# GoogleCloudPlatform/plspm-python

Measured on AMD Instinct MI355X. Metric: bootstrap replicates/sec (6-LV satisfaction model, N=10k), higher is better.
Workload: dtype f64

## Files before the change

plspm-python_amd/csrc/solver_wave16.h:

```cpp
#pragma once
#include "solver_wave.h"

namespace plspm {

template <int LMAX> struct W16 { static constexpr int VP = LMAX + 1; static constexpr bool TCOPY = LMAX <= 8; };

template <int LMAX>
struct Wave16Ws {
    double* stage;
    double* V;
    double* w;
    double* mu;
    double *Qm, *Gm, *Em;
    double* a;
    double* sink;
    double* scr;
    double* inv;
};
template <int LMAX> PLSPM_HD constexpr long wave16_v_doubles() {
    return (W16<LMAX>::TCOPY ? 2 : 1) * 64 * W16<LMAX>::VP > 16 * 66 ? (W16<LMAX>::TCOPY ? 2 : 1) * 64 * W16<LMAX>::VP : 16 * 66;
}
template <int LMAX> PLSPM_HD constexpr long wave16_ws_doubles(int L, int kmax, int n_chol = 0) { return wave16_v_doubles<LMAX>() + 64 + 64 + 3 * LMAX * LMAX + 2 * LMAX + (long)L * regression_scratch_doubles(kmax) + n_chol / 2; }
template <int LMAX> PLSPM_HD void wave16_carve(Wave16Ws<LMAX>& ws, double* base, int L, int kmax) {
    static_assert(LMAX == 32 || LMAX == 16 || LMAX == 8, "pair lane: column t mod LMAX, rows t / LMAX + (64 / LMAX) u");
    double* p = base;
    ws.stage = p; ws.V = p; p += wave16_v_doubles<LMAX>();
    ws.w = p; p += 64; ws.mu = p; p += 64;
    ws.Qm = p; p += LMAX * LMAX; ws.Gm = p; p += LMAX * LMAX; ws.Em = p; p += LMAX * LMAX;
    ws.a = p; p += LMAX; ws.sink = p; p += LMAX;
    ws.scr = p; p += (long)L * regression_scratch_doubles(kmax);
    ws.inv = p;
}
template <int LMAX> PLSPM_HD bool wave16_solver_covers(int P, int L, int n_chol, int kmax) {
    return P >= 1 && P <= 64 && L > LMAX / 2 && L <= LMAX && n_chol / 2 <= 16 * 66 && wave16_ws_doubles<LMAX>(L, kmax, n_chol) * (long)sizeof(double) <= (LMAX > 16 ? 53 : 40) * 1024;
}

struct NmWaveIo {
    double* maps;
    int force_T;
    int* steps;
    double bound_scale = 1.0;
};

template <int LMAX, bool MODEB = false, bool NM = false, class Ex>
PLSPM_HD void solve_problem_wave16(Ex& ex, const ModelDesc& md, const Wave16Ws<LMAX>& ws, const double* Md, const FitOutputs& out, const NmWaveIo* io = nullptr, double* nmk = nullptr) {
    constexpr int PMAX = 64, NE = LMAX * LMAX / 64;
    const int P = md.P, L = md.L, PS = cov_ld(P), t = ex.tid, p = t;
    const bool valid = p < P;
    const int pc = valid ? p : P - 1;
    const int lp = md.lvof[pc];
    const int em = t % LMAX, er0 = t / LMAX;
    const bool lvlane = t < L;
    unsigned dsc[NE];
#pragma unroll
    for (int u = 0; u < NE; ++u) {
        const int el = er0 + (64 / LMAX) * u;
        const bool pr = el < L && em < L;
        const int elc = pr ? el : 0, emc = pr ? em : 0;
        const int b0 = md.boff[elc];
        dsc[u] = (unsigned)b0 | (unsigned)(pr ? md.boff[elc + 1] - b0 : 0) << 8 | (unsigned)(pr ? (int)md.C[elc * L + emc] + 2 * (int)md.C[emc * L + elc] : 0) << 16 |
                 (pr ? 1u : 0u) << 24;
    }
    unsigned dl[NE];
#pragma unroll
    for (int u = 0; u < NE; ++u) dl[u] = dsc[u];
    auto pb0 = [&](int u) { return (int)(dl[u] & 255u); };
    auto pk = [&](int u) { return (int)((dl[u] >> 8) & 255u); };
    auto dlm = [&](int u) { return (int)((dl[u] >> 16) & 3u); };
    auto pairu = [&](int u) { return (dl[u] >> 24) != 0u; };
    int nk = 0;
    unsigned fpack = 0u;
    if (lvlane) {
        const int o = md.pred_off[t];
        nk = md.pred_off[t + 1] - o;
        for (int r = 0; r < 4; ++r) if (r < nk) fpack |= (unsigned)md.pred_idx[o + r] << (8 * r);
    }
    const int ne = md.n_eff;
    const double shp = md.scaled ? md.shift[pc] : 0.0;
    int kbmax = 0, kbB = 0;
    unsigned long long ends = 0ull;
    for (int l = 0; l < L; ++l) {
        const int k = md.boff[l + 1] - md.boff[l];
        kbmax = k > kbmax ? k : kbmax;
        if (MODEB && md.mode[l] == MODE_B) kbB = k > kbB ? k : kbB;
        ends |= 1ull << (md.boff[l + 1] - 1);
    }
    ends = ex.uniform(ends);
    bool singular = false;

    ex.mark(0);
    double s[PMAX];
    double dpp = 0.0, mup = 0.0;
    const double n = ex.uniform_d(Md[(long)P * PS + P]);
    ex.template load_cov<PMAX>(Md, PS, P, s, ws.stage, mup, dpp);
    if (!valid) { mup = 0.0; dpp = 0.0; }
    ex.mark(1);
    const double inv_n = ex.uniform_d(1.0 / n);
    const double sdraw = NM ? nm_column_sd(dpp * inv_n, mup * inv_n) : 1.0;
    ws.mu[p] = mup;
    ws.w[p] = NM ? (valid ? sdraw : 1.0) : 1.0;
    ex.sync();
    double fac = inv_n;
    if (!NM && md.scaled) {
        const double tot = ex.allsum(valid ? mup + n * shp : 0.0);
        const double np_ = n * (double)P, grand = tot / np_;
        const double d = shp - grand;
        const double ss = ex.allsum(valid ? dpp + 2.0 * d * mup + n * d * d : 0.0);
        const double g2 = ss / (np_ - 1.0) * ((n - 1.0) / n);
        fac = ex.uniform_d(1.0 / (n * g2));
    }
    ex.fence();
#pragma unroll
    for (int qb = 0; qb < PMAX; qb += 8) {
#pragma unroll
        for (int q = qb; q < qb + 8; ++q) {
            double v;
            if constexpr (NM) v = ((s[q] - (mup * ex.bcast(mup, (q < P) ? q : P - 1, ws.mu)) * inv_n) * inv_n) / (sdraw * ex.bcast(sdraw, (q < P) ? q : P - 1, ws.w));
            else v = (s[q] - (mup * ex.bcast(mup, (q < P) ? q : P - 1, ws.mu)) * inv_n) * fac;
            s[q] = (q < P) ? v : 0.0;
        }
        ex.pin8(s[qb], s[qb + 1], s[qb + 2], s[qb + 3], s[qb + 4], s[qb + 5], s[qb + 6], s[qb + 7]);
    }
    if (!valid) {
#pragma unroll
        for (int q = 0; q < PMAX; ++q) s[q] = 0.0;
    }
    const double sdp = NM ? sqrt(((dpp - (mup * mup) * inv_n) * inv_n) / (sdraw * sdraw)) : treated_sd(dpp, mup, inv_n, fac);
    if constexpr (!NM) {
        if (ex.vote_any(valid && sdp == 0.0)) {
            const double keep = (sdp == 0.0) ? 0.0 : 1.0;
#pragma unroll
            for (int q = 0; q < PMAX; ++q) s[q] *= keep;
        }
    }
    const double corr2 = ex.uniform_d(n / (n - 1.0));
    ex.mark(2);

    const bool modeb = MODEB && valid && md.mode[lp] == MODE_B;
    const int bb0 = md.boff[lp], bk = md.boff[lp + 1] - bb0, bi = p - bb0;
    const long boffB = modeb ? md.chol_off[lp] / 2 : 0;
    if constexpr (MODEB) {
        ex.sync();
        ws.mu[p] = (sdp > 0.0) ? sdp * sdp : 1e300;
        double* A = (kbB & 1) ? ws.stage : ws.inv;
        double* An = (kbB & 1) ? ws.inv : ws.stage;
        auto fill_block = [&](double* dst) {
#pragma unroll
            for (int q = 0; q < PMAX; ++q)
                if (modeb && q >= bb0 && q < bb0 + bk) dst[boffB + bi * bk + (q - bb0)] = s[q];
        };
        auto fill_block_all = [&](double* dst) {
            double* mine_row = dst + boffB + bi * bk - bb0;
            double* junk = ws.stage + 2 * LMAX * 16 + p;
            const unsigned bkm = modeb ? (unsigned)bk : 0u;
#pragma unroll
            for (int q = 0; q < PMAX; ++q) {
                double* d = ((unsigned)(q - bb0) < bkm) ? mine_row + q : junk;
                *d = s[q];
            }
        };
        bool okrow = true;
        ex.mark(20);
        auto sweep_rows = [&](auto krc) {
            constexpr int KR = decltype(krc)::value;
            fill_block_all(ws.inv);
            ex.sync();
            ex.mark(21);
            double row[KR];
            {
                const double* Ib0 = ws.inv + boffB + bi * bk;
#pragma unroll
                for (int c = 0; c < KR; ++c) row[c] = (modeb && c < bk) ? Ib0[c] : 0.0;
            }
            ex.mark(22);
            for (int j = 0; j < kbB; ++j) {
                double* Pj = ws.stage + ((j & 1) * LMAX + lp) * 16;
                if (modeb && bi == j) {
#pragma unroll
                    for (int c = 0; c < KR; ++c) Pj[c] = row[c];
                }
                ex.sync();
                if (modeb && j < bk) {
                    double f = 0.0;
#pragma unroll
                    for (int c = 0; c < KR; ++c) f = (c == j) ? row[c] : f;
                    const double piv = Pj[j];
                    okrow = okrow && (piv > PLSPM_PIVOT_RTOL * ws.mu[bb0 + j]);
                    const double ip = wave_rcp(piv);
                    const bool pivlane = bi == j;
                    const double fip = f * ip;
#pragma unroll
                    for (int c = 0; c < KR; ++c) {
                        const double rjc = Pj[c] * ip;
                        const double off = pivlane ? rjc : row[c] - f * rjc;
                        const double dia = pivlane ? ip : -fip;
                        row[c] = (c == j) ? dia : off;
                    }
                }
            }
            ex.mark(23);
#pragma unroll
            for (int c = 0; c < KR; ++c) if (modeb && c < bk) ws.inv[boffB + bi * bk + c] = row[c];
            ex.sync();
            ex.mark(24);
        };
        if (kbB <= 8) sweep_rows(std::integral_constant<int, 8>{});
        else if (kbB <= 12) sweep_rows(std::integral_constant<int, 12>{});
        else if (kbB <= 16) sweep_rows(std::integral_constant<int, 16>{});
        else {
        fill_block(A);
        ex.sync();
        for (int j = 0; j < kbB; ++j) {
            if (modeb) {
                const double* Ab = A + boffB;
                double* Ob = An + boffB;
                if (j < bk) {
                    const double piv = Ab[j * bk + j];
                    okrow = okrow && (piv > PLSPM_PIVOT_RTOL * ws.mu[bb0 + j]);
                    const double ip = 1.0 / piv;
                    const double f = Ab[bi * bk + j];
                    for (int c = 0; c < bk; ++c) {
                        const double rjc = Ab[j * bk + c] * ip;
                        double v;
                        if (bi == j) v = (c == j) ? ip : rjc;
                        else v = (c == j) ? -f * ip : Ab[bi * bk + c] - f * rjc;
                        Ob[bi * bk + c] = v;
                    }
                } else {
                    for (int c = 0; c < bk; ++c) Ob[bi * bk + c] = Ab[bi * bk + c];
                }
            }
            ex.sync();
            double* t = A; A = An; An = t;
        }
        }
        const bool any_bad = ex.vote_any(modeb && !okrow);
        for (int l = 0; any_bad && l < L; ++l) {
            if (md.mode[l] != MODE_B) continue;
            const int k = md.boff[l + 1] - md.boff[l];
            const bool bad_here = ex.vote_any(modeb && lp == l && !okrow);
            if (!bad_here) continue;
            if (lp == l) fill_block(ws.inv);
            ex.sync();
            if (p == l) {
                double* F = ws.inv + md.chol_off[l] / 2;
                bool ok = k > 1 && jacobi_pinv(F, k, ws.stage);
                if (!ok) singular = true;
                for (int r = 0; r < k; ++r) for (int c = 0; c < r; ++c) F[r * k + c] = F[c * k + r];
            }
            ex.sync();
        }
        ex.mark(25);
    }


    const int* fglob = md.pred_idx + (lvlane ? md.pred_off[t] : 0);
    const long rscr = regression_scratch_doubles(md.kmax);
    const int km = md.kmax;
    auto pred = [&](int r) { return r < 4 ? (int)((fpack >> (8 * r)) & 255u) : fglob[r]; };
    auto regress = [&](const double* M) {
        double* scratch = ws.scr + t * rscr;
        double* x = scratch + 2 * km * km;
        bool ok;
        if (nk <= 4) {
            unsigned fp = fpack;
            ex.opaque(fp);
            ok = wave_ldl4(M, LMAX, fp, nk, t, x);
        } else {
            for (int r = 0; r < nk; ++r) {
                for (int c = 0; c < nk; ++c) scratch[r * nk + c] = M[fglob[r] * LMAX + fglob[c]];
                x[r] = M[fglob[r] * LMAX + t];
            }
            ok = chol_factor(scratch, nk);
            if (ok) chol_solve(scratch, nk, x);
        }
        if (!ok && !(nk > 1 && pinv_solve(M, LMAX, fglob, nk, t, x, scratch))) singular = true;
        return x;
    };

    const double icorr2 = ex.uniform_d((n - 1.0) / n);
    double Qe[NE], wp = valid ? 1.0 : 0.0;
#pragma unroll
    for (int u = 0; u < NE; ++u) Qe[u] = 0.0;
    int iteration = 0, phase = 0;
    double a_prev = 0.0, Ra_prev = 0.0;
    if constexpr (NM) {
        ex.sync();
        wp = valid ? 1.0 / sqrt((double)(md.boff[lp + 1] - md.boff[lp])) : 0.0;
        ws.w[p] = valid ? wp : 1.0;
        ex.sync();
        phase = 1;
    }
    while (true) {
        int pl = p, lpl = lp;
        ex.opaque(pl); ex.opaque(lpl);
#pragma unroll
        for (int u = 0; u < NE; ++u) { dl[u] = dsc[u]; ex.opaque(dl[u]); }
        const int eml = pl % LMAX, er0l = pl / LMAX;
        ex.mark(16);
        if constexpr (W16<LMAX>::TCOPY) ex.template seg_products2<PMAX, 64 * W16<LMAX>::VP * 8>(s, ws.w, P, ends, ws.V + pl * W16<LMAX>::VP, wp);
        else ex.template seg_products<PMAX>(s, ws.w, P, ends, valid ? ws.V + pl * W16<LMAX>::VP : ex.sink(ws.sink));
        ex.mark(17);
        ex.sync();
        ex.mark(18);
        if constexpr (NE == 1) {
            double s0 = 0.0, s1 = 0.0;
            int pb = pb0(0);
            ex.opaque(pb);
            const double* vv = ws.V + pb * W16<LMAX>::VP + eml;
            const double* ww = ws.w + pb;
            for (int i0 = 0; i0 < kbmax; i0 += 8) {
                double v[8];
#pragma unroll
                for (int j = 0; j < 8; ++j) {
                    if constexpr (W16<LMAX>::TCOPY) v[j] = (i0 + j < pk(0)) ? vv[(64 + i0 + j) * W16<LMAX>::VP] : 0.0;
                    else v[j] = (i0 + j < pk(0)) ? ww[i0 + j] * vv[(i0 + j) * W16<LMAX>::VP] : 0.0;
                }
                s0 += v[0]; s1 += v[1]; s0 += v[2]; s1 += v[3]; s0 += v[4]; s1 += v[5]; s0 += v[6]; s1 += v[7];
            }
            Qe[0] = s0 + s1;
            ws.Qm[pl] = pairu(0) ? Qe[0] : 1.0;
        } else {
            double s0[NE], s1[NE];
#pragma unroll
            for (int u = 0; u < NE; ++u) { s0[u] = 0.0; s1[u] = 0.0; }
            auto terms = [&](auto ttc) {
                constexpr int TT = decltype(ttc)::value;
                for (int i0 = 0; i0 < kbmax; i0 += TT) {
#pragma unroll
                    for (int u = 0; u < NE; ++u) {
                        if ((64 / LMAX) * u < L) {
                            const int pb = pb0(u), pkk = pk(u);
                            const double* vv = ws.V + pb * W16<LMAX>::VP + eml;
                            const double* ww = ws.w + pb;
                            double v[TT];
#pragma unroll
                            for (int j = 0; j < TT; ++j) v[j] = (i0 + j < pkk) ? ww[i0 + j] * vv[(i0 + j) * W16<LMAX>::VP] : 0.0;
#pragma unroll
                            for (int j = 0; j < TT; j += 2) { s0[u] += v[j]; s1[u] += v[j + 1]; }
                        }
                    }
                }
            };
            if (kbmax <= (NE <= 4 ? 4 : 2)) terms(std::integral_constant<int, (NE <= 4 ? 4 : 2)>{});
            else if (NE > 4) terms(std::integral_constant<int, 4>{});
            else {
#pragma unroll
                for (int u = 0; u < NE; ++u) {
                    if ((64 / LMAX) * u < L) {
                        int pb = pb0(u);
                        ex.opaque(pb);
                        const int pkk = pk(u);
                        const double* vv = ws.V + pb * W16<LMAX>::VP + eml;
                        const double* ww = ws.w + pb;
                        for (int i0 = 0; i0 < kbmax; i0 += 8) {
                            double v[8];
#pragma unroll
                            for (int j = 0; j < 8; ++j) v[j] = (i0 + j < pkk) ? ww[i0 + j] * vv[(i0 + j) * W16<LMAX>::VP] : 0.0;
                            s0[u] += v[0]; s1[u] += v[1]; s0[u] += v[2]; s1[u] += v[3]; s0[u] += v[4]; s1[u] += v[5]; s0[u] += v[6]; s1[u] += v[7];
                        }
                    }
                }
            }
#pragma unroll
            for (int u = 0; u < NE; ++u) {
                if ((64 / LMAX) * u < L) {
                    Qe[u] = s0[u] + s1[u];
                    ws.Qm[pl + 64 * u] = pairu(u) ? Qe[u] : 1.0;
                }
            }
        }
        ex.sync();
        ex.mark(19);
        bool nm_first = false;
        if constexpr (NM) {
            nm_first = iteration == 0;
            const double wfl = nm_first ? 1.0 : wave_rsqrt(ws.Qm[lpl * LMAX + lpl]);
            const double a_cur = valid ? wp * wfl : 0.0, Ra_cur = valid ? ws.V[pl * W16<LMAX>::VP + lpl] * wfl : 0.0;
            bool stop = false;
            double ub = 0.0;
            if (!nm_first) {
                const double d = a_cur - a_prev, Rd = Ra_cur - Ra_prev;
                ub = n * ex.allsum(d * Rd);
                stop = (io && io->force_T > 0) ? (iteration >= io->force_T) : (ub * (io ? io->bound_scale : 1.0) < md.tol * (1.0 - 1e-9));
                if (iteration > md.max_iter) stop = true;
            }
            if (stop) break;
            a_prev = a_cur; Ra_prev = Ra_cur;
            const double cmap = a_cur / sdraw;
            if (io && io->maps && valid) io->maps[(long)iteration * (P + L + 1) + pl] = cmap;
            if (io && io->maps && pl == 0) io->maps[(long)iteration * (P + L + 1) + P + L] = ub;
            nmk[pl] = valid ? (mup * inv_n) * cmap : 0.0;
        }
        if (!NM && phase == 2) break;
        if (phase == 0) {
            wp = valid ? wave_rsqrt(ws.Qm[lpl * LMAX + lpl]) : 0.0;
            ws.w[pl] = valid ? wp : 1.0;
            ex.sync();
            ex.mark(3);
            phase = 1;
            continue;
        }
        ++iteration;
        ex.mark(9);
        const double rm = wave_rsqrt(ws.Qm[eml * LMAX + eml]), am = NM ? (nm_first ? 1.0 : rm) : rm * icorr2;
#pragma unroll
        for (int u = 0; u < NE; ++u) {
            if ((64 / LMAX) * u < L) {
                const int ell = er0l + (64 / LMAX) * u;
                const double rl = wave_rsqrt(ws.Qm[ell * LMAX + ell]), al = NM ? (nm_first ? 1.0 : rl) : rl * icorr2;
                const double Ge = al * am * Qe[u];
                double Ee = 0.0;
                if (pairu(u)) {
                    if (md.scheme == SCHEME_PATH) {
                        if (dlm(u) & 1) Ee = Qe[u] * rl * rm;
                    } else if (dlm(u)) {
                        const int d = (dlm(u) & 1) + (dlm(u) >> 1);
                        Ee = (md.scheme == SCHEME_CENTROID) ? ((Ge > 0.0) ? 1.0 : ((Ge < 0.0) ? -1.0 : 0.0)) : Ge * corr2 * (double)d;
                    }
                    ws.Gm[pl + 64 * u] = Ge; ws.Em[pl + 64 * u] = al * Ee;
                    if (ell == eml) ws.a[ell] = al;
                }
            }
        }
        ex.sync();
        ex.mark(10);
        if constexpr (NM) {
            if (io && io->maps && lvlane) {
                double k0 = 0.0;
                for (int q = md.boff[pl]; q < md.boff[pl + 1]; ++q) k0 += nmk[q];
                io->maps[(long)(iteration - 1) * (P + L + 1) + P + pl] = -k0;
            }
        }
        if (md.scheme == SCHEME_PATH) {
            if (lvlane && nk > 0) {
                const double* x = regress(ws.Gm);
#pragma unroll
                for (int r = 0; r < 4; ++r) if (r < nk) ws.Em[pred(r) * LMAX + pl] = ws.a[pred(r)] * x[r];
                for (int r = 4; r < nk; ++r) ws.Em[pred(r) * LMAX + pl] = ws.a[pred(r)] * x[r];
            }
            ex.sync();
        }
        ex.mark(11);
        double c0 = 0.0, c1 = 0.0;
#pragma unroll
        for (int m = 0; m + 1 < LMAX; m += 2) {
            if (m < L) c0 += ws.V[pl * W16<LMAX>::VP + m] * ws.Em[m * LMAX + lpl];
            if (m + 1 < L) c1 += ws.V[pl * W16<LMAX>::VP + m + 1] * ws.Em[(m + 1) * LMAX + lpl];
        }
        double wn = valid ? c0 + c1 : 0.0;
        if constexpr (MODEB) {
            ws.mu[pl] = wn;
            ex.sync();
            if (modeb) {
                const double* Ib = ws.inv + boffB + bi * bk;
                const double* cb = ws.mu + bb0;
                double a0 = 0.0, a1 = 0.0;
                int q = 0;
                for (; q + 1 < bk; q += 2) { a0 += Ib[q] * cb[q]; a1 += Ib[q + 1] * cb[q + 1]; }
                if (q < bk) a0 += Ib[q] * cb[q];
                wn = a0 + a1;
            }
        }
        if constexpr (NM) {
            wp = wn;
            ws.w[pl] = valid ? wp : 1.0;
            ex.sync();
            ex.mark(12);
        } else {
        const double dd = fabs(wp) - fabs(wn);
        const double conv = ex.allsum(dd * dd);
        wp = wn;
        ws.w[pl] = valid ? wp : 1.0;
        ex.sync();
        ex.mark(12);
        if (conv < md.tol || iteration > md.max_iter) phase = 2;
        }
    }
    const bool not_converged = iteration > md.max_iter;
    ex.mark(4);

    const double wfp = wave_rsqrt(ws.Qm[lp * LMAX + lp]);
    wp *= wfp;
    unsigned negmask = 0u;
    {
        double vr[LMAX];
#pragma unroll
        for (int l = 0; l < LMAX; ++l) vr[l] = ws.V[p * W16<LMAX>::VP + (l < L ? l : 0)];
#pragma unroll
        for (int l = 0; l < LMAX; ++l)
            if (!NM && l < L) { const int neg = ex.vote_count(valid && vr[l] < 0.0 && sdp != 0.0); if (P - 2 * neg < 0) negmask |= 1u << l; }
    }
    const double sgl = ((negmask >> lp) & 1u) ? -1.0 : 1.0;
    const double vlp = ws.V[p * W16<LMAX>::VP + lp];
    double* const Cs = ws.Gm;
    double* const Bm = ws.Em;
    double* const Ind = ws.Qm;
    {
        const double wfm = wave_rsqrt(ws.Qm[em * LMAX + em]), sm = ((negmask >> em) & 1u) ? -1.0 : 1.0;
        double cs[NE];
#pragma unroll
        for (int u = 0; u < NE; ++u) {
            const int el = er0 + (64 / LMAX) * u;
            const double wfl = wave_rsqrt(ws.Qm[el * LMAX + el]), sl = ((negmask >> el) & 1u) ? -1.0 : 1.0;
            cs[u] = sl * sm * wfl * wfm * Qe[u];
        }
#pragma unroll
        for (int u = 0; u < NE; ++u) {
            if (pairu(u)) Cs[t + 64 * u] = cs[u];
            Bm[t + 64 * u] = 0.0;
        }
    }
    ex.sync();
    ex.mark(5);
    double r2p = 0.0;
    if (lvlane) {
        if (nk > 0) {
            const double* x = regress(Cs);
            double expl = 0.0;
#pragma unroll
            for (int r = 0; r < 4; ++r)
                if (r < nk) { const int fr = pred(r); Bm[t * LMAX + fr] = x[r]; expl += x[r] * Cs[fr * LMAX + t]; }
            for (int r = 4; r < nk; ++r) { const int fr = pred(r); Bm[t * LMAX + fr] = x[r]; expl += x[r] * Cs[fr * LMAX + t]; }
            r2p = expl / Cs[t * LMAX + t];
        }
    }
    ex.sync();
    ex.mark(6);
    if (lvlane) {
        double colx[LMAX];
#pragma unroll
        for (int i = 0; i < LMAX; ++i) {
            double i0 = 0.0, i1 = 0.0;
#pragma unroll
            for (int k = 0; k + 1 < i; k += 2) { i0 += Bm[i * LMAX + k] * colx[k]; i1 += Bm[i * LMAX + k + 1] * colx[k + 1]; }
            if (i & 1) i0 += Bm[i * LMAX + i - 1] * colx[i - 1];
            const double ind = (i > t) ? i0 + i1 : 0.0;
            colx[i] = (i > t) ? Bm[i * LMAX + t] + ind : 0.0;
            Ind[i * LMAX + t] = ind;
        }
    }
    ex.sync();
    ex.mark(7);
    if (out.row) {
        if (valid) {
            out.row[p] = wp;
            out.row[P + L + 2 * ne + p] = (sdp > 0.0) ? sgl * vlp * wfp / sdp : 0.0;
        }
        if (lvlane) out.row[P + t] = r2p;
        for (int e = t; e < ne; e += 64) {
            const int idx = md.eff_to[e] * LMAX + md.eff_from[e];
            out.row[P + L + e] = Bm[idx] + Ind[idx];
            out.row[P + L + ne + e] = Bm[idx];
        }
    }
    const bool bad = ex.vote_any((valid && !(isfinite(wp) && isfinite(sdp) && sdp >= 0.0)) || (lvlane && !isfinite(r2p)));
    const bool sing = ex.vote_any(singular);
    if (t == 0) {
        int st = sing ? ST_SINGULAR : (not_converged ? ST_NOT_CONVERGED : ST_OK);
        if (st == ST_OK && bad) st = ST_NONFINITE;
        if (out.status) *out.status = st;
        if (out.iters) *out.iters = iteration;
        if (out.row) { out.row[2 * P + L + 2 * ne] = (double)st; out.row[2 * P + L + 2 * ne + 1] = (double)iteration; }
        if constexpr (NM) { if (io && io->steps) *io->steps = iteration; }
    }
    ex.mark(13);
}

}
```

Measured before the change: 10.71 million.

## Fold covariance centering into segment products for LMAX=8 wave solver

For the LMAX=8 mode-A non-NM path, the explicit centering and scaling of the 64-entry covariance row is skipped, along with the zero-variance masking pass. Instead the mean correction is applied algebraically afterwards, to the LV covariance entries, the outer weights and the loadings, using an extra column-sum row stored in V. This removes the per-row O(PMAX) rescale work and one barrier. In exchange it adds some extra reductions and shared-memory traffic, and it risks cancellation error because the raw, uncentered moments are used.

```diff
diff --git a/plspm-python_amd/csrc/solver_wave16.h b/plspm-python_amd/csrc/solver_wave16.h
--- a/plspm-python_amd/csrc/solver_wave16.h
+++ b/plspm-python_amd/csrc/solver_wave16.h
@@ -45,6 +45,8 @@
 template <int LMAX, bool MODEB = false, bool NM = false, class Ex>
 PLSPM_HD void solve_problem_wave16(Ex& ex, const ModelDesc& md, const Wave16Ws<LMAX>& ws, const double* Md, const FitOutputs& out, const NmWaveIo* io = nullptr, double* nmk = nullptr) {
     constexpr int PMAX = 64, NE = LMAX * LMAX / 64;
+    constexpr bool FOLD = LMAX == 8 && !MODEB && !NM;
+    constexpr int VP = W16<LMAX>::VP;
     const int P = md.P, L = md.L, PS = cov_ld(P), t = ex.tid, p = t;
     const bool valid = p < P;
     const int pc = valid ? p : P - 1;
@@ -97,9 +99,11 @@
     ex.mark(1);
     const double inv_n = ex.uniform_d(1.0 / n);
     const double sdraw = NM ? nm_column_sd(dpp * inv_n, mup * inv_n) : 1.0;
-    ws.mu[p] = mup;
-    ws.w[p] = NM ? (valid ? sdraw : 1.0) : 1.0;
-    ex.sync();
+    if constexpr (!FOLD) {
+        ws.mu[p] = mup;
+        ws.w[p] = NM ? (valid ? sdraw : 1.0) : 1.0;
+        ex.sync();
+    }
     double fac = inv_n;
     if (!NM && md.scaled) {
         const double tot = ex.allsum(valid ? mup + n * shp : 0.0);
@@ -110,6 +114,13 @@
         fac = ex.uniform_d(1.0 / (n * g2));
     }
     ex.fence();
+    const double* const cc = (P < PMAX) ? ws.V + P * VP : ws.sink;
+    const double mupn = mup * inv_n;
+    if constexpr (FOLD) {
+#if !defined(__HIP_DEVICE_COMPILE__)
+        if (t == P) for (int q = 0; q < P; ++q) s[q] = Md[(long)q * PS + P];
+#endif
+    } else {
 #pragma unroll
     for (int qb = 0; qb < PMAX; qb += 8) {
 #pragma unroll
@@ -125,8 +136,15 @@
 #pragma unroll
         for (int q = 0; q < PMAX; ++q) s[q] = 0.0;
     }
+    }
     const double sdp = NM ? sqrt(((dpp - (mup * mup) * inv_n) * inv_n) / (sdraw * sdraw)) : treated_sd(dpp, mup, inv_n, fac);
-    if constexpr (!NM) {
+    const bool live = FOLD ? (valid && sdp != 0.0) : valid;
+    if constexpr (FOLD) {
+        ws.w[p] = valid ? (live ? 1.0 : 0.0) : 1.0;
+        if (P == PMAX) ws.mu[p] = live ? mupn * n : 0.0;
+        ex.sync();
+    }
+    if constexpr (!NM && !FOLD) {
         if (ex.vote_any(valid && sdp == 0.0)) {
             const double keep = (sdp == 0.0) ? 0.0 : 1.0;
 #pragma unroll
@@ -279,7 +297,7 @@
     };
 
     const double icorr2 = ex.uniform_d((n - 1.0) / n);
-    double Qe[NE], wp = valid ? 1.0 : 0.0;
+    double Qe[NE], wp = live ? 1.0 : 0.0;
 #pragma unroll
     for (int u = 0; u < NE; ++u) Qe[u] = 0.0;
     int iteration = 0, phase = 0;
@@ -299,7 +317,14 @@
         const int eml = pl % LMAX, er0l = pl / LMAX;
         ex.mark(16);
         if constexpr (W16<LMAX>::TCOPY) ex.template seg_products2<PMAX, 64 * W16<LMAX>::VP * 8>(s, ws.w, P, ends, ws.V + pl * W16<LMAX>::VP, wp);
-        else ex.template seg_products<PMAX>(s, ws.w, P, ends, valid ? ws.V + pl * W16<LMAX>::VP : ex.sink(ws.sink));
+        else ex.template seg_products<PMAX>(s, ws.w, P, ends, (FOLD ? pl <= P : valid) ? ws.V + pl * W16<LMAX>::VP : ex.sink(ws.sink));
+        if constexpr (FOLD) {
+            if (P == PMAX && lvlane) {
+                double c0 = 0.0;
+                for (int q = md.boff[pl]; q < md.boff[pl + 1]; ++q) c0 += ws.mu[q];
+                ws.sink[pl] = c0;
+            }
+        }
         ex.mark(17);
         ex.sync();
         ex.mark(18);
@@ -319,6 +344,7 @@
                 s0 += v[0]; s1 += v[1]; s0 += v[2]; s1 += v[3]; s0 += v[4]; s1 += v[5]; s0 += v[6]; s1 += v[7];
             }
             Qe[0] = s0 + s1;
+            if constexpr (FOLD) Qe[0] = (Qe[0] - (cc[er0l] * cc[eml]) * inv_n) * fac;
             ws.Qm[pl] = pairu(0) ? Qe[0] : 1.0;
         } else {
             double s0[NE], s1[NE];
@@ -366,6 +392,7 @@
             for (int u = 0; u < NE; ++u) {
                 if ((64 / LMAX) * u < L) {
                     Qe[u] = s0[u] + s1[u];
+                    if constexpr (FOLD) Qe[u] = (Qe[u] - (cc[er0l + (64 / LMAX) * u] * cc[eml]) * inv_n) * fac;
                     ws.Qm[pl + 64 * u] = pairu(u) ? Qe[u] : 1.0;
                 }
             }
@@ -394,8 +421,9 @@
         }
         if (!NM && phase == 2) break;
         if (phase == 0) {
-            wp = valid ? wave_rsqrt(ws.Qm[lpl * LMAX + lpl]) : 0.0;
+            wp = live ? wave_rsqrt(ws.Qm[lpl * LMAX + lpl]) : 0.0;
             ws.w[pl] = valid ? wp : 1.0;
+            if constexpr (FOLD) { if (P == PMAX) ws.mu[pl] = (mupn * n) * wp; }
             ex.sync();
             ex.mark(3);
             phase = 1;
@@ -442,13 +470,18 @@
             ex.sync();
         }
         ex.mark(11);
-        double c0 = 0.0, c1 = 0.0;
+        double c0 = 0.0, c1 = 0.0, e0 = 0.0, e1 = 0.0;
+        double cv[FOLD ? LMAX : 1];
+        if constexpr (FOLD) {
+#pragma unroll
+            for (int m = 0; m < LMAX; ++m) cv[m] = cc[m];
+        }
 #pragma unroll
         for (int m = 0; m + 1 < LMAX; m += 2) {
-            if (m < L) c0 += ws.V[pl * W16<LMAX>::VP + m] * ws.Em[m * LMAX + lpl];
-            if (m + 1 < L) c1 += ws.V[pl * W16<LMAX>::VP + m + 1] * ws.Em[(m + 1) * LMAX + lpl];
-        }
-        double wn = valid ? c0 + c1 : 0.0;
+            if (m < L) { const double e = ws.Em[m * LMAX + lpl]; c0 += ws.V[pl * VP + m] * e; if constexpr (FOLD) e0 += cv[m] * e; }
+            if (m + 1 < L) { const double e = ws.Em[(m + 1) * LMAX + lpl]; c1 += ws.V[pl * VP + m + 1] * e; if constexpr (FOLD) e1 += cv[m + 1] * e; }
+        }
+        double wn = FOLD ? (live ? ((c0 + c1) - mupn * (e0 + e1)) * fac : 0.0) : (valid ? c0 + c1 : 0.0);
         if constexpr (MODEB) {
             ws.mu[pl] = wn;
             ex.sync();
@@ -472,6 +505,7 @@
         const double conv = ex.allsum(dd * dd);
         wp = wn;
         ws.w[pl] = valid ? wp : 1.0;
+        if constexpr (FOLD) { if (P == PMAX) ws.mu[pl] = (mupn * n) * wp; }
         ex.sync();
         ex.mark(12);
         if (conv < md.tol || iteration > md.max_iter) phase = 2;
@@ -487,12 +521,16 @@
         double vr[LMAX];
 #pragma unroll
         for (int l = 0; l < LMAX; ++l) vr[l] = ws.V[p * W16<LMAX>::VP + (l < L ? l : 0)];
+        if constexpr (FOLD) {
+#pragma unroll
+            for (int l = 0; l < LMAX; ++l) vr[l] -= mupn * cc[l < L ? l : 0];
+        }
 #pragma unroll
         for (int l = 0; l < LMAX; ++l)
             if (!NM && l < L) { const int neg = ex.vote_count(valid && vr[l] < 0.0 && sdp != 0.0); if (P - 2 * neg < 0) negmask |= 1u << l; }
     }
     const double sgl = ((negmask >> lp) & 1u) ? -1.0 : 1.0;
-    const double vlp = ws.V[p * W16<LMAX>::VP + lp];
+    const double vlp = FOLD ? (ws.V[p * VP + lp] - mupn * cc[lp]) * fac : ws.V[p * VP + lp];
     double* const Cs = ws.Gm;
     double* const Bm = ws.Em;
     double* const Ind = ws.Qm;
```

After: 10.74 million, median of 6. No clear change (+0.3%).
